# Daffan/legged_tracking

Measured on AMD Instinct MI355X. Metric: env-steps/sec (whole node) at 4096 Go1/GPU, 1/2/4/8 MI355X; %HBM roofline, higher is better.
Workload: dtype f32

## Files before the change

legged_tracking_amd/csrc/go1_contact.h:

```cpp
#pragma once
#ifndef GO1_DEVICE_H
#error "include go1_device.h: its parts are not self-contained"
#endif
#pragma clang fp contract(on)

#define PSZX 20
#define PSZY 16
static_assert(PSZY == 16 && PSZX % 2 == 0, "the LDS-DMA patch staging maps 2 rows of 16 cells to a wave");
struct Terr {
  const float* tile;
  int nx, ny;
  float hs;
  const float2* patch;
  int pi0, pj0;
};

__device__ __forceinline__ float tile_at(const Terr& T, int layer, int i, int j) {
  i = min(max(i, 0), T.nx - 1);
  j = min(max(j, 0), T.ny - 1);
  return T.tile[((size_t)layer * T.nx + i) * T.ny + j];
}

struct CP {
  float k, d, kf, mu;
// ... 311 lines not shown
      ymin = fminf(ymin, pp[1]); ymax = fmaxf(ymax, pp[1]);
    }
    float sn, cn;
    __sincosf(q[j], &sn, &cn);
#pragma unroll
    for (int a = 0; a < 3; ++a) rE(j == 0 ? 0 : 1, cn, sn, Rp + 3 * a, Rp + 3 * a);
  }
  float fw[3];
  mat3_vec(Rp, GO1_MODEL_F32 + 13 * 10 + 4 * 9, fw);
  const float fx = pp[0] + fw[0], fy = pp[1] + fw[1];
  xmin = quad_min(fminf(xmin, fx)); xmax = quad_max(fmaxf(xmax, fx));
  ymin = quad_min(fminf(ymin, fy)); ymax = quad_max(fmaxf(ymax, fy));
  *cx = 0.5f * (xmin + xmax);
  *cy = 0.5f * (ymin + ymax);
}

#define FACE_Q 1.0e-5f
#define FACE_W 10
__device__ __forceinline__ int face_key_max(int v) {
  v = max(v, __builtin_amdgcn_update_dpp(0, v, 0xB1, 0xF, 0xF, true));
  v = max(v, __builtin_amdgcn_update_dpp(0, v, 0x4E, 0xF, 0xF, true));
  auto a = __builtin_amdgcn_permlane16_swap((uint32_t)v, (uint32_t)v, false, false);
  v = max((int)a[0], (int)a[1]);
  auto b = __builtin_amdgcn_permlane32_swap((uint32_t)v, (uint32_t)v, false, false);
  return max((int)b[0], (int)b[1]);
}
#define FACE_SIGNED 0.1f
__device__ __forceinline__ void face_scan(const Terr& T, const float* R, const float* pos, const float* th, int sub16,
                                          int* sel) {
  const float ihs = frcp(T.hs);
  const int ci = (int)floorf(fminf(fmaxf(pos[0] * ihs, -16000.0f), 16000.0f));
  const int cj = (int)floorf(fminf(fmaxf(pos[1] * ihs, -16000.0f), 16000.0f));
  int key[2] = {-1, -1};
#pragma unroll
  for (int u = 0; u < (FACE_W * FACE_W + 15) / 16; ++u) {
    const int v = sub16 + 16 * u;
    const int i = ci + v % FACE_W - 4, j = cj + v / FACE_W - 4;
    const int li = i - T.pi0, lj = j - T.pj0;
    const bool inp = (v < FACE_W * FACE_W) & (li >= 0) & (li < PSZX) & (lj >= 0) & (lj < PSZY);
    const float2 hv = T.patch[min(max(li, 0), PSZX - 1) * PSZY + min(max(lj, 0), PSZY - 1)];
    const float dx = (float)i * T.hs - pos[0], dy = (float)j * T.hs - pos[1];
    const f2 dz = f2{hv.x, hv.y} - pos[2];
    const f2 cx = (R[0] * dx + R[3] * dy) + R[6] * dz, cy = (R[1] * dx + R[4] * dy) + R[7] * dz,
             cz = (R[2] * dx + R[5] * dy) + R[8] * dz;
    const f2 pen = f2{cz.x + th[2], th[2] - cz.y};
#pragma unroll
    for (int hh = 0; hh < 2; ++hh) {
      const bool in = inp & (fabsf(cx[hh]) <= th[0]) & (fabsf(cy[hh]) <= th[1]) & (pen[hh] > -FACE_SIGNED);
      const int q = (int)floorf(fminf(pen[hh] + FACE_SIGNED, 10.0f) * (1.0f / FACE_Q));
      const int k = in ? (q << 7) | (127 - v) : -1;
      key[hh] = max(key[hh], k);
    }
  }
#pragma unroll
  for (int hh = 0; hh < 2; ++hh) {
    const int k = face_key_max(key[hh]);
    const int v = 127 - (k & 127);
    const int i = ci + v % FACE_W - 4, j = cj + v / FACE_W - 4;
    sel[hh] = k < 0 ? -1 : ((i + 16384) << 16) | (j + 16384);
  }
}
__device__ __forceinline__ void face_force(const Terr& T, const CP& C, const float* R, const float* pos, const float* vb,
                                           const float* th, const int* sel, f2* w, float* Fw) {
  f2 cx, cy, cz;
  bool ok[2];
#pragma unroll
  for (int hh = 0; hh < 2; ++hh) {
    const int i = (sel[hh] >> 16) - 16384, j = (sel[hh] & 0xffff) - 16384;
    const int li = i - T.pi0, lj = j - T.pj0;
    ok[hh] = sel[hh] >= 0 & li >= 0 & li < PSZX & lj >= 0 & lj < PSZY;
    const float2 hv = T.patch[min(max(li, 0), PSZX - 1) * PSZY + min(max(lj, 0), PSZY - 1)];
    const float dx = (float)i * T.hs - pos[0], dy = (float)j * T.hs - pos[1], dz = (hh == 0 ? hv.x : hv.y) - pos[2];
    cx[hh] = (R[0] * dx + R[3] * dy) + R[6] * dz;
// ... 30 lines not shown
```

legged_tracking_amd/csrc/go1_phys.h:

```cpp
#pragma once
#ifndef GO1_DEVICE_H
#error "include go1_device.h: its parts are not self-contained"
#endif
#pragma clang fp contract(on)

#define LDS_DDP (GO1_MODEL_FLOATS)
#define LDS_DPL (LDS_DDP + 12)
#define LDS_TL (LDS_DPL + 24)
#define LDS_HL (LDS_TL + 12)
#define LDS_GX (LDS_HL + 24)
#define LDS_GY (LDS_GX + GO1_GRID_X)
#define LDS_FLOATS (LDS_GY + GO1_GRID_Y)
static_assert(offsetof(go1_config, height_grid_y) - offsetof(go1_config, default_dof_pos) ==
                  (LDS_GY - LDS_DDP) * sizeof(float),
              "per-joint config arrays must be contiguous in go1_config");

struct Phys {
  float pos[3], quat[4];
  f2 wv[3];
  float q[3], qd[3];
};

__device__ __forceinline__ void phys_substep(CCfg* __restrict__ cfg, const float* lds, Phys& S, const float* tau,
                                             float h, const float* g, float friction, float restitution,
                                             float payload, const Terr& T, int leg, int role, bool cf_out,
                                             float* cf_raw, float* self_sc, bool face_scan_now) {
#pragma clang fp contract(on)
  (void)lds;
  const float* model = GO1_MODEL_F32;
  const float msx = (leg & 2) ? -1.0f : 1.0f, msy = (leg & 1) ? -1.0f : 1.0f, msxy = msx * msy;
  float LC[39];
#pragma unroll
  for (int i = 0; i < 39; ++i) {
    const int p = GO1_LEG_SIGN[i];
    LC[i] = p == 0 ? GO1_LEG_FL[i] : GO1_LEG_FL[i] * (p == 1 ? msx : (p == 2 ? msy : msxy));
  }
  MARK(phys_begin);
  const CP C = {cfg->contact_stiffness, cfg->contact_damping, cfg->friction_damping, friction,
                0.5f * (restitution + cfg->terrain_restitution), cfg->bounce_threshold};
  float R[9];
  quat_to_R(S.quat, R);
  f2 vbp[3];
#pragma unroll
  for (int i = 0; i < 3; ++i) vbp[i] = R[i] * S.wv[0] + R[3 + i] * S.wv[1] + R[6 + i] * S.wv[2];
  const float vb[6] = {vbp[0].x, vbp[1].x, vbp[2].x, vbp[0].y, vbp[1].y, vbp[2].y};
  const float* th = model + 13 * 10 + 4 * 9 + 3 + 1;
#ifndef GO1_ABL_NO_FACES
  if (T.patch && face_scan_now) {
    int sel[2];
    face_scan(T, R, S.pos, th, 4 * role + leg, sel);
    if (role == 0 && leg == 0) {
      int* fsel = reinterpret_cast<int*>(self_sc + FACE_SEL_OFF);
      fsel[0] = sel[0];
      fsel[1] = sel[1];
    }
    asm volatile("s_waitcnt lgkmcnt(0)" ::: "memory");
  }
#endif
  const float* origin = LC + 30;
  const float* foot = model + 13 * 10 + 4 * 9;
  const float foot_r = foot[3];
  const float thigh_r = model[13 * 10 + 4 * 9 + 3 + 1 + 3];
  const float calf_r = model[13 * 10 + 4 * 9 + 3 + 1 + 3 + 1];
  const float hip_r = model[13 * 10 + 4 * 9 + 3 + 1 + 3 + 2];
  const float hip_y0 = model[13 * 10 + 4 * 9 + 3 + 1 + 3 + 3], hip_y1 = model[13 * 10 + 4 * 9 + 3 + 1 + 3 + 4];
  float cs[3][2];
  const bool even = (role & 1) == 0;
  f2 Rs[9], ps[3], vs[6];
#pragma unroll
  for (int i = 0; i < 9; ++i) Rs[i] = f2{0.0f, R[i]};
#pragma unroll
  for (int i = 0; i < 3; ++i) { ps[i] = f2{0.0f, S.pos[i]}; vs[i] = f2{0.0f, vb[i]}; vs[3 + i] = f2{0.0f, vb[3 + i]}; }
  float pth[3], pkn[3], pft[3];
  f2 cjp[3][3], pAp[3][3];
  {
    f2 R01[3], pp01 = f2{S.pos[0], S.pos[1]};
    float R2[3], pp2 = S.pos[2];
    f2 vp[3];
#pragma unroll
    for (int k = 0; k < 3; ++k) { R01[k] = f2{R[k], R[3 + k]}; R2[k] = R[6 + k]; }
#pragma unroll
    for (int i = 0; i < 3; ++i) vp[i] = vbp[i];
#pragma unroll
    for (int j = 0; j < 3; ++j) {
      const int ax = j == 0 ? 0 : 1;
      const float* r = origin + j * 3;
      float sn, cn;
      hw_sincosf(S.q[j], &sn, &cn);
      cs[j][0] = cn; cs[j][1] = sn;
      f2 vj[3];
// ... 44 lines not shown
#pragma unroll
      for (int i = 0; i < 3; ++i) vp[i] = vj[i];
    }
  }
  MARK(leg_kin_done);
  float fx[6], fy[6], fbase[6];
  f2 Fpt[3];
  float Fo[3] = {0.0f, 0.0f, 0.0f};
  float Fbs[3] = {0.0f, 0.0f, 0.0f};
  SIP cin[2];
#ifndef GO1_ABL_NO_CONTACT
  {
    f2 lpA[3], lpB[3], rr;
    {
      const float* kn = origin + 6;
      const int cA = leg * 2, cB = leg * 2 + 1;
      const float crn[2][3] = {{(cA & 1) ? th[0] : -th[0], (cA & 2) ? th[1] : -th[1], (cA & 4) ? th[2] : -th[2]},
                               {(cB & 1) ? th[0] : -th[0], (cB & 2) ? th[1] : -th[1], (cB & 4) ? th[2] : -th[2]}};
#pragma unroll
      for (int i = 0; i < 3; ++i) {
        const float hyA = i == 1 ? msy * hip_y0 : 0.0f, hyB = i == 1 ? msy * hip_y1 : 0.0f;
        const float xa = sel4(role, 0.0f, hyA, 0.0f, foot[i]);
        const float xb = sel4(role, 0.5f * kn[i], hyB, 0.5f * foot[i], foot[i]);
        const float ya = sel4(role, kn[i], crn[0][i], foot[i], crn[1][i]);
        const float yb = sel4(role, 0.5f * kn[i], crn[0][i], 0.5f * foot[i], crn[1][i]);
        lpA[i] = f2{xa, ya};
        lpB[i] = f2{xb, yb};
      }
      rr = f2{sel4(role, thigh_r, hip_r, calf_r, foot_r), sel4(role, thigh_r, 0.0f, calf_r, 0.0f)};
    }
    float wb[6] = {0.0f, 0.0f, 0.0f, 0.0f, 0.0f, 0.0f}, Mo[3] = {0.0f, 0.0f, 0.0f};
    MARK(self_begin);
#ifndef GO1_ABL_NO_SELF
    const bool self_on = cfg->self_stiffness > 0.0f;
    int mask;
    {
      const f2 hy = msy * f2{hip_y0, hip_y1};
      const f2 hcy = origin[1] + cs[0][0] * hy, hcz = origin[2] + cs[0][1] * hy;
      const float hc0[3] = {origin[0], hcy.x, hcz.x}, hc1[3] = {origin[0], hcy.y, hcz.y};
      mask = self_broad(leg, pth, pkn, pft, fmaxf(foot_r, fmaxf(thigh_r, calf_r)), hc0, hc1, hip_r, R, S.pos, th,
                        S.q);
      mask = self_on ? mask : 0;
    }
#else
    const bool self_on = false;
    const int mask = 0;
#endif
    MARK(self_broad_done);
#ifdef GO1_ABL_NO_NARROW
    if (__any(mask != 0) && mask == 12345) {
#else
    if (__any(mask != 0)) {
#endif
      float P0[3], P1[3];
      f2 e[3];
      {
        const float* kn = origin + 6;
#pragma unroll
        for (int i = 0; i < 3; ++i) {
          const float hy0 = i == 1 ? msy * hip_y0 : 0.0f, hy1 = i == 1 ? msy * hip_y1 : 0.0f;
          e[i] = f2{sel4(role, 0.0f, hy0, 0.0f, foot[i]), sel4(role, kn[i], hy1, foot[i], foot[i])};
        }
#pragma unroll
        for (int i = 0; i < 3; ++i) {
          const f2 p = ps[i].x + Rs[3 * i].x * e[0] + Rs[3 * i + 1].x * e[1] + Rs[3 * i + 2].x * e[2];
          P0[i] = p.x; P1[i] = p.y;
        }
// ... 2 lines not shown
        const float w[3] = {vs[0].x, vs[1].x, vs[2].x};
        const f2 wl[3] = {w[1] * e[2] - w[2] * e[1], w[2] * e[0] - w[0] * e[2], w[0] * e[1] - w[1] * e[0]};
        const f2 vlin[3] = {vs[3].x + wl[0], vs[4].x + wl[1], vs[5].x + wl[2]};
#pragma unroll
        for (int i = 0; i < 3; ++i) {
          const f2 v = Rs[3 * i].x * vlin[0] + Rs[3 * i + 1].x * vlin[1] + Rs[3 * i + 2].x * vlin[2];
          V0[i] = v.x; V1[i] = v.y;
        }
      };
      const float half = sel4(role, 0.5f * fabsf(origin[8]), 0.5f * (hip_y1 - hip_y0), 0.5f * fabsf(foot[2]), 0.0f);
      self_put(self_sc, leg, role, P0, P1, rr.x, half + rr.x);
      static_assert(TPB == 64, "self-collision LDS exchange assumes one wave per block");
      asm volatile("s_waitcnt lgkmcnt(0)" ::: "memory");
      MARK(self_put_done);
      const float pb[3] = {ps[0].x, ps[1].x, ps[2].x};
      float own_lo[3], own_hi[3];
#pragma unroll
      for (int i = 0; i < 3; ++i) { own_lo[i] = fminf(P0[i], P1[i]) - rr.x; own_hi[i] = fmaxf(P0[i], P1[i]) + rr.x; }
      self_narrow(cfg, self_sc, leg, role, mask, R, S.pos, vb, th, pb, own_lo, own_hi, Fo, Mo, wb, vel);
      asm volatile("s_waitcnt lgkmcnt(0)" ::: "memory");
      MARK(self_narrow_done);
    }
    f2 lp[3], pw[3], vw[3];
    HQ qa, qb;
    int cell[2];
    {
      f2 wA[3], wB[3];
#pragma unroll
      for (int i = 0; i < 3; ++i) {
        wA[i] = ps[i] + Rs[3 * i] * lpA[0] + Rs[3 * i + 1] * lpA[1] + Rs[3 * i + 2] * lpA[2];
        wB[i] = ps[i] + Rs[3 * i] * lpB[0] + Rs[3 * i + 1] * lpB[1] + Rs[3 * i + 2] * lpB[2];
      }
      MARK(seg_begin);
      float2* held = reinterpret_cast<float2*>(self_sc + SEG_T_OFF) + (4 * role + leg);
      f2 ts;
      if (face_scan_now) {
#ifdef GO1_ABL_NO_WALK
        ts = f2{0.0f, 0.0f} * (wA[0] + wB[0]);
        cell[0] = SEG_CELL((int)floorf(wA[0].x / T.hs), (int)floorf(wA[1].x / T.hs), false);
        cell[1] = SEG_CELL((int)floorf(wA[0].y / T.hs), (int)floorf(wA[1].y / T.hs), false);
#else
        ts = seg_deepest2(T, wA, wB, rr, cell);
#endif
        *held = make_float2(ts.x, ts.y);
      } else {
        const float2 hv = *held;
        ts = f2{hv.x, hv.y};
      }
      MARK(seg_done);
#pragma unroll
      for (int i = 0; i < 3; ++i) lp[i] = lpA[i] + ts * (lpB[i] - lpA[i]);
      const f2 wl[3] = {vs[1] * lp[2] - vs[2] * lp[1], vs[2] * lp[0] - vs[0] * lp[2], vs[0] * lp[1] - vs[1] * lp[0]};
      const f2 vlin[3] = {vs[3] + wl[0], vs[4] + wl[1], vs[5] + wl[2]};
#pragma unroll
      for (int i = 0; i < 3; ++i) {
        pw[i] = ps[i] + Rs[3 * i] * lp[0] + Rs[3 * i + 1] * lp[1] + Rs[3 * i + 2] * lp[2];
        vw[i] = Rs[3 * i] * vlin[0] + Rs[3 * i + 1] * vlin[1] + Rs[3 * i + 2] * vlin[2];
      }
    }
    if (face_scan_now) {
      hq_fetch_cell(T, pw[0].x, pw[1].x, cell[0], qa);
      hq_fetch_cell(T, pw[0].y, pw[1].y, cell[1], qb);
    } else {
      hq_fetch(T, pw[0].x, pw[1].x, qa);
      hq_fetch(T, pw[0].y, pw[1].y, qb);
    }
    float Fa[3], Fb2[3], Ma[6], Mb[6];
    {
      const float pa[3] = {pw[0].x, pw[1].x, pw[2].x}, va[3] = {vw[0].x, vw[1].x, vw[2].x};
      const float pb[3] = {pw[0].y, pw[1].y, pw[2].y}, vb2[3] = {vw[0].y, vw[1].y, vw[2].y};
      sphere_contact_im(T, qa, C, pa, va, rr.x, h, Fa, Ma);
      sphere_contact_im(T, qb, C, pb, vb2, rr.y, h, Fb2, Mb);
    }
    if (self_on) {
#pragma unroll
      for (int i = 0; i < 3; ++i) Fbs[i] = R[3 * i] * wb[3] + R[3 * i + 1] * wb[4] + R[3 * i + 2] * wb[5];
    }
    const f2 F[3] = {f2{Fa[0], Fb2[0]}, f2{Fa[1], Fb2[1]}, f2{Fa[2], Fb2[2]}};
    f2 Fd[3];
#pragma unroll
// ... 156 lines not shown
      for (int a = 0; a < 3; ++a)
#pragma unroll
        for (int b = 0; b < 3; ++b) Ia.b[a * 3 + b] = IA.b[a * 3 + b] - Up[j][a].x * V[b].y;
      f2 Iac[3], pa[3], pt[3];
      sip_mul_sparse(Ia, cjp[j], ax, Iac);
      const float ud = u[j] * invD;
#pragma unroll
      for (int i = 0; i < 3; ++i) pa[i] = pAp[j][i] + Iac[i] + Up[j][i] * ud;
      SIP It;
      xform_inertia2(ax, cs[j][0], cs[j][1], offset_mask(j), origin + j * 3, Ia, It);
      xfT2(ax, cs[j][0], cs[j][1], offset_mask(j), origin + j * 3, pa, pt);
      if (j > 0) {
        rigid_sip(LC + 10 * (j - 1), 1.0f, IA);
        sip_add(IA, It);
        sip_add(IA, j == 2 ? ci_th : ci_hp);
#pragma unroll
        for (int i = 0; i < 3; ++i) pAp[j - 1][i] += pt[i];
      } else {
        Ip = It;
        sip_add(Ip, ci_bs);
#pragma unroll
        for (int i = 0; i < 3; ++i) pp6[i] = pt[i];
      }
    }
  }
  MARK(backward_done);
  f2 wface[3] = {f2{0.0f, 0.0f}, f2{0.0f, 0.0f}, f2{0.0f, 0.0f}};
  float Fface[3] = {0.0f, 0.0f, 0.0f};
#ifdef GO1_ABL_NO_FACES
  if (false) {
#else
  if (T.patch) {
#endif
    const int* fsel = reinterpret_cast<const int*>(self_sc + FACE_SEL_OFF);
    const int sel[2] = {fsel[0], fsel[1]};
    face_force(T, C, R, S.pos, vb, th, sel, wface, Fface);
  }
  MARK(faces_done);
  const float* bb = model;
  const float mscale = (bb[0] + payload) * frcp(bb[0]);
  SIP I0;
  rigid_sip(bb, mscale, I0);
  f2 p0[3];
  float gb[3];
  rigid_bias2(bb, vbp, p0, mscale);
  mat3T_vec(R, g, gb);
#pragma unroll
  for (int k = 0; k < 6; ++k) Ip.ac[k] = f2{qsum(Ip.ac[k].x), qsum(Ip.ac[k].y)};
#pragma unroll
  for (int i = 0; i < 3; ++i) pp6[i] = f2{qsum(pp6[i].x - fbase[i]), qsum(pp6[i].y - fbase[3 + i])} - wface[i];
#pragma unroll
  for (int i = 0; i < 9; ++i) Ip.b[i] = qsum(Ip.b[i]);
  sip_add(I0, Ip);
  float rhs[6], a0[6];
#pragma unroll
  for (int i = 0; i < 3; ++i) {
    rhs[i] = -(p0[i].x + pp6[i].x);
    rhs[3 + i] = -(p0[i].y + pp6[i].y);
  }
#ifdef GO1_ABL_NO_BASESOLVE
#pragma unroll
  for (int i = 0; i < 6; ++i) a0[i] = rhs[i] * 0.05f;
  (void)I0;
#else
#ifdef GO1_ABL_NO_CHOL
  float tr = 0.0f;
#pragma unroll
  for (int k = 0; k < 6; ++k) tr += I0.ac[k].x + I0.ac[k].y;
#pragma unroll
// ... 96 lines not shown
```

legged_tracking_amd/csrc/go1_selfcol.h:

```cpp
#pragma once
#ifndef GO1_DEVICE_H
#error "include go1_device.h: its parts are not self-contained"
#endif
#pragma clang fp contract(on)

#define SELF_ENV_FLOATS (16 * 16 + 4 + 32)
#define FACE_SEL_OFF (16 * 16)
#define SEG_T_OFF (16 * 16 + 4)

__device__ __forceinline__ void self_put(float* sc, int leg, int role, const float* P0, const float* P1, float r,
                                         float rb) {
  float4* Q = reinterpret_cast<float4*>(sc) + 4 * (4 * leg + role);
  Q[0] = make_float4(P0[0], P0[1], P0[2], r);
  Q[1] = make_float4(P1[0], P1[1], P1[2], rb);
}
__device__ __forceinline__ void self_put_vel(float* sc, int leg, int role, const float* V0, const float* V1) {
  float4* Q = reinterpret_cast<float4*>(sc) + 4 * (4 * leg + role);
  Q[2] = make_float4(V0[0], V0[1], V0[2], 0.0f);
  Q[3] = make_float4(V1[0], V1[1], V1[2], 0.0f);
}

__device__ __forceinline__ void seg_closest(const float* P0, const float* d1, const float* Q0, const float* d2,
                                            float& s, float& t) {
  const float r[3] = {P0[0] - Q0[0], P0[1] - Q0[1], P0[2] - Q0[2]};
  const float a = d1[0] * d1[0] + d1[1] * d1[1] + d1[2] * d1[2], e = d2[0] * d2[0] + d2[1] * d2[1] + d2[2] * d2[2];
  const float b = d1[0] * d2[0] + d1[1] * d2[1] + d1[2] * d2[2];
  const float c = d1[0] * r[0] + d1[1] * r[1] + d1[2] * r[2], f = d2[0] * r[0] + d2[1] * r[1] + d2[2] * r[2];
  float n[3], m[3];
  cross3(d1, d2, n);
  cross3(d2, r, m);
  const float den = n[0] * n[0] + n[1] * n[1] + n[2] * n[2], num = n[0] * m[0] + n[1] * m[1] + n[2] * m[2];
  const bool pa = a > 1e-12f, pe = e > 1e-12f;
  const float ia = pa ? frcp(a) : 0.0f, ie = pe ? frcp(e) : 0.0f;
  const float s0 = den > 1e-10f * a * e ? __builtin_amdgcn_fmed3f(num * frcp(den), 0.0f, 1.0f) : 0.0f;
  const float tt = (b * s0 + f) * ie;
  const float s_lo = __builtin_amdgcn_fmed3f(-c * ia, 0.0f, 1.0f), s_hi = __builtin_amdgcn_fmed3f((b - c) * ia, 0.0f, 1.0f);
  const float ss = tt < 0.0f ? s_lo : (tt > 1.0f ? s_hi : s0);
  const float t_pt = __builtin_amdgcn_fmed3f(f * ie, 0.0f, 1.0f);
  s = !pa ? 0.0f : (!pe ? s_lo : ss);
  t = !pe ? 0.0f : (!pa ? t_pt : __builtin_amdgcn_fmed3f(tt, 0.0f, 1.0f));
}
// ... 274 lines not shown
```

legged_tracking_amd/csrc/go1_spec.h:

```cpp
#pragma once
#define GO1_SPEC_FIELDS(X) \
  X(terrain_kind, 1) \
  X(camera_zero, 1) \
  X(measure_front_half, 1) \
  X(add_noise, 1) \
  X(use_terminal_body_height, 1) \
  X(rand_interval, 300) \
  X(hf_nx, 80) \
  X(hf_ny, 40) \
  X(n_terms, 10) \
  X(term_mask, 23647u) \
  X(reward_mode, 0) \
  X(lin_vel_form, 0) \
  X(terminate_end_of_trajectory, 0) \
  X(use_terminal_body_rotation, 0) \
  X(rotate_camera, 0) \
  X(observe_heights, 1) \
  X(timestep_in_obs, 0) \
  X(num_obs, 261) \
  X(u_per_env, 308) \
  X(traj_kind, 0) \
  X(traj_length, 1) \
  X(traj_interp, 1) \
  X(indefinite_slots, 0u) \
  X(live_slots, 1023u) \
  X(sigma_rew_neg, 0x1.4000000000000p+2f) \
  X(small_vel_threshold, 0x1.99999a0000000p-4f) \
  X(large_dist_threshold, 0x0.0p+0f) \
  X(dt, 0x1.47ae140000000p-6f) \
  X(action_scale, 0x1.0000000000000p-2f) \
  X(hip_scale_reduction, 0x1.0000000000000p-1f) \
  X(clip_actions, 0x1.4000000000000p+3f) \
  X(clip_obs, 0x1.9000000000000p+6f) \
  X(horizontal_scale, 0x1.99999a0000000p-5f) \
// ... 33 lines not shown
#define GO1_SPEC_action_scale 0x1.0000000000000p-2f
#define GO1_SPEC_hip_scale_reduction 0x1.0000000000000p-1f
#define GO1_SPEC_clip_actions 0x1.4000000000000p+3f
#define GO1_SPEC_clip_obs 0x1.9000000000000p+6f
#define GO1_SPEC_horizontal_scale 0x1.99999a0000000p-5f
#define GO1_SPEC_max_episode_length 0x1.f400000000000p+8f
#define GO1_SPEC_terminal_body_height 0x0.0p+0f
#define GO1_SPEC_switch_dist 0x1.3333340000000p-2f
#define GO1_SPEC_base_height_target 0x1.1eb8520000000p-2f
#define GO1_SPEC_tracking_sigma_lin 0x1.99999a0000000p-5f
#define GO1_SPEC_tracking_sigma_ang 0x1.0000000000000p-1f
#define GO1_SPEC_target_lin_vel 0x1.0000000000000p-2f
#define GO1_SPEC_target_ang_vel 0x1.921fb60000000p+0f
#define GO1_SPEC_lin_reaching_criterion 0x1.3333340000000p-2f
#define GO1_SPEC_ang_reaching_criterion 0x1.41b2f80000000p-3f
#define GO1_SPEC_t_reach 0x0.0p+0f
#define GO1_SPEC_ceiling_height 0x1.99999a0000000p-1f
#define GO1_SPEC_obs_scale_dof_pos 0x1.0000000000000p+0f
#define GO1_SPEC_obs_scale_dof_vel 0x1.99999a0000000p-5f
#define GO1_SPEC_obs_scale_heights 0x1.99999a0000000p-4f
#define GO1_SPEC_noise_gravity 0x1.99999a0000000p-5f
#define GO1_SPEC_noise_dof_pos 0x1.47ae140000000p-7f
#define GO1_SPEC_noise_dof_vel 0x1.3333340000000p-4f
#define GO1_SPEC_camera_offset_x 0x1.eb851e0000000p-4f
#define GO1_SPEC_camera_offset_norm 0x1.eb851e0000000p-4f
#define GO1_SPEC_priv_friction_shift 0x1.0000000000000p-1f
#define GO1_SPEC_priv_friction_scale 0x1.0000000000000p+1f
#define GO1_SPEC_priv_rest_shift 0x1.0000000000000p-1f
#define GO1_SPEC_priv_rest_scale 0x1.0000000000000p+1f
#define GO1_SPEC_strength_range 0x1.99999a0000000p-3f
#define GO1_SPEC_strength_lo 0x1.cccccc0000000p-1f
#define GO1_SPEC_offset_range 0x1.47ae140000000p-5f
#define GO1_SPEC_offset_lo -0x1.47ae140000000p-6f
#define GO1_SPEC_terrain_kind 1
#define GO1_SPEC_camera_zero 1
#define GO1_SPEC_measure_front_half 1
#define GO1_SPEC_add_noise 1
#define GO1_SPEC_use_terminal_body_height 1
#define GO1_SPEC_rand_interval 300
#define GO1_SPEC_hf_nx 80
#define GO1_SPEC_hf_ny 40
#define GO1_SPEC_n_terms 10
#define GO1_SPEC_term_mask 23647u
#define GO1_SPEC_reward_mode 0
#define GO1_SPEC_lin_vel_form 0
#define GO1_SPEC_terminate_end_of_trajectory 0
#define GO1_SPEC_use_terminal_body_rotation 0
#define GO1_SPEC_rotate_camera 0
#define GO1_SPEC_observe_heights 1
#define GO1_SPEC_timestep_in_obs 0
#define GO1_SPEC_num_obs 261
#define GO1_SPEC_u_per_env 308
#define GO1_SPEC_traj_kind 0
#define GO1_SPEC_traj_length 1
#define GO1_SPEC_traj_interp 1
#define GO1_SPEC_indefinite_slots 0u
#define GO1_SPEC_live_slots 1023u
```

legged_tracking_amd/csrc/go1_step.hip:

```cpp
#include "go1_device.h"
#include "go1_step_shared.h"

#define HOLD_N 23

struct KArgs {
  go1_state st;
  go1_terrain ter;
  go1_step_args a;
  int32_t* flags;
  int cur, prv, nxt;
  const uint8_t* prev_time_out;
  uint8_t* prev_extras;
  float* bucket_r;
  double* bucket_sum;
};

__device__ void traj_waypoint(CCfg* __restrict__ c, const Rng& rng, const float* root, int w, float* o) {
  const int ub = GO1_U_NOISE + c->num_obs;
  if (c->traj_kind == 1) {
    const int ni = c->traj_interp, nt = c->traj_length / ni + 1, sg = w / ni, j = w % ni;
    const float rng_of[6] = {c->traj_x_range, c->traj_y_range, c->traj_z_range, c->traj_yaw_range,
                             c->traj_pitch_range, c->traj_roll_range};
    const int out_of[6] = {0, 1, 2, 5, 4, 3};
#pragma unroll
// ... 211 lines not shown
        const int tix_s = __builtin_amdgcn_readlane(tix, 4 * el2);
        const int pi_s = __builtin_amdgcn_readlane(T.pi0, 4 * el2);
        const int pj_s = __builtin_amdgcn_readlane(T.pj0, 4 * el2);
        const float* tl = K.ter.tiles + (size_t)tix_s * 2 * nx * ny;
        const int gj = min(max(pj_s + cj, 0), ny - 1);
#pragma unroll
        for (int k = 0; k < PSZX / 2; ++k) {
          const int gi = min(max(pi_s + 2 * k + ci_l, 0), nx - 1);
          __builtin_amdgcn_global_load_lds(tl + (layer_off + gi) * ny + gj, (float*)&s_patch[el2][0] + 64 * k, 4, 0, 0);
        }
      }
    }
  }
  MARK(pro_dma_issued);
  __shared__ float s_hold[HOLD_N][TPB];
  auto hold = [&](bool park) {
    int hl = lane;
    if (!park) asm volatile("" : "+v"(hl));
    float* hp = &s_hold[0][hl];
    auto f = [&](int k, float& v) { if (park) hp[k * TPB] = v; else v = hp[k * TPB]; };
    auto i = [&](int k, int& v) { float x = __int_as_float(v); f(k, x); v = __float_as_int(x); };
#pragma unroll
    for (int k = 0; k < 6; ++k) f(k, traj_in[k]);
#pragma unroll
    for (int k = 0; k < 3; ++k) { f(6 + k, ldv[k]); f(9 + k, la[k]); f(12 + k, eo_pre[k]); }
    f(15, cam_pitch); f(16, my_scale); f(17, my_sum); f(18, my_tot);
    i(19, ep_in); i(20, idx_in); i(21, coll_in); i(22, my_id);
  };
  hold(true);
  asm volatile("" : "+v"(rebind_flag));
  if (rebind && sub16 == 0 && rebind_flag) K.prev_extras[e] = rebind_val;

  float cf_raw[CF_RAW] = {0, 0, 0, 0, 0, 0, 0, 0, 0}, cf_leg[9], cf_base[3], cf_hip[3];
  step_substeps<INJ>(c, A, J, P, s_mlp, s_phys, T, s_self[el], cf_raw, KL, friction, restitution, payload, e, lane,
                     CI(action_scale), CI(hip_scale_reduction), leg, role);
  contact_totals<INJ>(cf_raw, A.inj_contact, e, leg, role, cf_leg, cf_base, cf_hip);
  hold(false);
  float root[13];
  if (INJ) {
#pragma unroll
    for (int i = 0; i < 13; ++i) root[i] = A.inj_root[(size_t)e * 13 + i];
  } else {
    phys_store_root(P, root);
    root[0] = P.pos[0] + org_x;
    root[1] = P.pos[1] + org_y;
  }
  const bool hplane = CI(terrain_kind) == 0;
  const float scan_x = root[0], scan_y = root[1];
  const float cam_p = CI(rotate_camera) ? 0.0f : cam_pitch;
  float camx = 0.0f, camy = 0.0f;
  if (!hplane) {
    const float cos_p = pm_cosf(cam_p);
    camx = CI(camera_offset_x) * cos_p;
    camy = 0.0f * cos_p;
  }
  auto sample = [&](int i, int j, float& h0, float& h1) {
    if (hplane) { h0 = 1.0f; h1 = 0.0f; return; }
    float px, py;
    if constexpr (STREAM) {
      px = c_gen->scan_x[i] + scan_x;
      py = c_gen->scan_y[j] + scan_y;
    } else {
      px = s_phys[LDS_GX + i] + scan_x;
      py = s_phys[LDS_GY + j] + scan_y;
    }
    if (CI(camera_zero)) { px = px + camx; py = py + camy; }
    px = px - org_x;
    py = py - org_y;
    const float fx = fminf(fmaxf(px / CI(horizontal_scale), -1.0f), (float)CI(hf_nx));
    const float fy = fminf(fmaxf(py / CI(horizontal_scale), -1.0f), (float)CI(hf_ny));
// ... 536 lines not shown
  go1_terrain ter;
  bool bound = false, has_terrain = false;
  int32_t* d_flags = nullptr;
  float* d_bucket_r = nullptr;
  double* d_bucket_sum = nullptr;
  uint64_t count = 0;
  bool spec = false;
  bool streamed = false;
  const uint8_t* prev_time_out = nullptr;
  uint8_t* prev_extras = nullptr;
};

static thread_local std::string g_err;

#define P(f, cols, dt) GO1_PLANE(go1_state, f, cols, GO1_DTYPE_##dt)
static const PlaneRow STATE_PLANES[] = {
    P(root, 13, F32), P(dof_pos, 12, F32), P(dof_vel, 12, F32), P(last_actions, 12, F32), P(last_dof_vel, 12, F32),
    P(lag, 0, F32), P(pos_err_hist, 24, F32), P(vel_hist, 24, F32), P(motor_strength, 12, F32),
    P(motor_offset, 12, F32), P(friction, 1, F32), P(restitution, 1, F32), P(payload, 1, F32),
    P(episode_length, 1, I32), P(curr_pose_index, 1, I32), P(trajectory, 0, F32), P(base_rotation, 3, F32),
    P(collision_count, 1, I32), P(episode_sums, 0, F32), P(joint_pos_target, 12, F32), P(feet_air_time, 4, F32),
    P(last_contacts, 4, F32)};
#undef P
static_assert(sizeof(STATE_PLANES) / sizeof(STATE_PLANES[0]) == GO1_STATE_PLANES &&
                  sizeof(go1_state) == GO1_STATE_PLANES * sizeof(void*), "go1_state planes");

template <class T>
static bool spec_eq(T a, T b) { return memcmp(&a, &b, sizeof(T)) == 0; }
static bool spec_match(const go1_config& c) {
  bool m = true;
#define GO1_SPEC_CHECK(f, v) m = m && spec_eq(c.f, (decltype(c.f))(v));
  GO1_SPEC_FIELDS(GO1_SPEC_CHECK)
#undef GO1_SPEC_CHECK
  return m && c.decimation == 4;
}
static bool scan_compiled_in(const go1_config& c) { return c.scan_nx == GO1_GRID_X && c.scan_ny == GO1_GRID_Y; }

static int fail(int code, const std::string& msg) {
  g_err = msg;
  return code;
}
#define HIP_TRY(x) GO1_HIP_TRY(fail, x)
int go1_internal_fail(int code, const std::string& msg) { return fail(code, msg); }

extern "C" {
#ifdef GO1_STAMPS
int go1_debug_stamps(void* host, size_t bytes) {
  if (bytes > sizeof(g_go1_stamps)) bytes = sizeof(g_go1_stamps);
  return hipMemcpyFromSymbol(host, HIP_SYMBOL(g_go1_stamps), bytes, 0, hipMemcpyDeviceToHost) == hipSuccess ? 0 : 1;
}
int go1_debug_stamps_clear(void) {
  void* p = nullptr;
  if (hipGetSymbolAddress(&p, HIP_SYMBOL(g_go1_stamps)) != hipSuccess) return 1;
  if (hipMemset(p, 0, sizeof(g_go1_stamps)) != hipSuccess) return 1;
  return hipDeviceSynchronize() == hipSuccess ? 0 : 1;
}
#endif

int go1_abi_version(void) { return GO1_ABI_VERSION; }

void go1_abi_sizes(int64_t out[4]) {
  out[0] = sizeof(go1_config);
  out[1] = sizeof(go1_state);
  out[2] = sizeof(go1_terrain);
  out[3] = sizeof(go1_step_args);
}

// ... 236 lines not shown
```

legged_tracking_amd/csrc/go1_step_shared.h:

```cpp
#pragma once
#include "go1_device.h"

#pragma clang fp contract(off)

template <int KMAX>
struct Joints {
  float (&act)[3], (&q)[3], (&qd)[3], (&eh)[2][3], (&vh)[2][3], (&strength)[3], (&offset)[3];
  float (&dflt)[3], (&tlim)[3], (&lag_pre)[KMAX][3];
  float (&scaled)[3], (&torque)[3], (&tgt)[3];
};

__device__ __forceinline__ void phys_load_root(Phys& P, const float* root) {
#pragma unroll
  for (int i = 0; i < 3; ++i) {
    P.pos[i] = root[i];
    P.wv[i] = f2{root[10 + i], root[7 + i]};
  }
#pragma unroll
  for (int i = 0; i < 4; ++i) P.quat[i] = root[3 + i];
}
__device__ __forceinline__ void phys_store_root(const Phys& P, float* root) {
#pragma unroll
  for (int i = 0; i < 3; ++i) {
    root[i] = P.pos[i]; root[7 + i] = P.wv[i].y; root[10 + i] = P.wv[i].x;
  }
#pragma unroll
  for (int i = 0; i < 4; ++i) root[3 + i] = P.quat[i];
}

template <bool INJ, int KMAX, class Args>
__device__ __forceinline__ void step_substeps(CCfg* c, const Args& A, const Joints<KMAX>& J, Phys& P,
                                              const float* s_mlp, const float* s_phys, const Terr& T, float* s_self,
                                              float* cf_raw, int KL, float friction, float restitution,
                                              float payload, int e, int lane, float action_scale,
                                              float hip_scale_reduction, int leg, int role) {
  const int lq = lane >> 4, n = c->n_envs, dec = c->decimation;
#pragma unroll
  for (int j = 0; j < 3; ++j) {
    J.scaled[j] = J.act[j] * action_scale;
    if (j == 0) J.scaled[j] = J.scaled[j] * hip_scale_reduction;
  }
  for (int sub = 0; sub < dec; ++sub) {
    MARK(sub_begin);
    {
      const int m = 6 - sub;
      const int back = m <= 0 ? 0 : (m + dec - 1) / dec;
      float xin[3][6];
#pragma unroll
      for (int j = 0; j < 3; ++j) {
        float lg = J.scaled[j];
#pragma unroll
        for (int k = 0; k < KMAX; ++k) lg = back == KL - k ? J.lag_pre[k][j] : lg;
        J.tgt[j] = lg + J.dflt[j];
        const float err = J.q[j] - J.tgt[j] + J.offset[j];
        xin[j][0] = err; xin[j][1] = J.eh[0][j]; xin[j][2] = J.eh[1][j];
        xin[j][3] = J.qd[j]; xin[j][4] = J.vh[0][j]; xin[j][5] = J.vh[1][j];
      }
      MARK(mlp_begin);
      float tq[3] = {0.0f, 0.0f, 0.0f};
      float b0[3], b1v[3];
#pragma unroll
      for (int j = 0; j < 3; ++j) {
        const float* y = xin[j];
        b0[j] = sel4(lq, y[0], y[1], y[2], y[3]);
        b1v[j] = sel4(lq, y[4], y[5], 0.0f, 0.0f);
      }
#ifdef GO1_ABL_NO_MLP
#pragma unroll
      for (int j = 0; j < 3; ++j) tq[j] = 0.0f * (b0[j] + b1v[j]);
#else
      {
        MlpFrag Fs;
        mlp_unpark(Fs, s_mlp, lane);
        mlp_group3(Fs, b0, b1v, tq);
      }
#endif
#ifdef GO1_ABL_NO_MLP
#pragma unroll
      for (int j = 0; j < 3; ++j) tq[j] += -20.0f * xin[j][0] - 0.5f * xin[j][3];
#endif
      MARK(mlp_done);
#pragma unroll
      for (int j = 0; j < 3; ++j) {
        J.eh[1][j] = J.eh[0][j];
        J.eh[0][j] = xin[j][0];
        J.vh[1][j] = J.vh[0][j];
        J.vh[0][j] = J.qd[j];
        const float t = tq[j] * J.strength[j];
        const float lim = J.tlim[j];
        J.torque[j] = clampf(t, -lim, lim);
      }
    }
    if (INJ) {
      const float* id = A.inj_dof + ((size_t)sub * n + e) * NDOF * 2;
#pragma unroll
      for (int j = 0; j < 3; ++j) {
        J.q[j] = id[(leg * 3 + j) * 2];
        J.qd[j] = id[(leg * 3 + j) * 2 + 1];
      }
    } else {
      const float h = c->sim_dt / (float)c->n_internal;
#pragma unroll
      for (int j = 0; j < 3; ++j) { P.q[j] = J.q[j]; P.qd[j] = J.qd[j]; }
      MARK(phys_call);
#ifndef GO1_ABL_NO_PHYS
      for (int k = 0; k < c->n_internal; ++k) {
        const bool last = (sub == dec - 1) && (k == c->n_internal - 1);
        phys_substep(c, s_phys, P, J.torque, h, A.sim_gravity, friction, restitution, payload, T, leg, role, last,
                     cf_raw, s_self, sub == 0 && k == 0);
      }
#else
      P.qd[0] += 1e-4f * J.torque[0]; P.qd[1] += 1e-4f * J.torque[1]; P.qd[2] += 1e-4f * J.torque[2];
#endif
#pragma unroll
      for (int j = 0; j < 3; ++j) { J.q[j] = P.q[j]; J.qd[j] = P.qd[j]; }
      MARK(phys_returned);
    }
    if (A.dbg_torques && role == 0) {
#pragma unroll
      for (int j = 0; j < 3; ++j) A.dbg_torques[((size_t)sub * n + e) * NDOF + leg * 3 + j] = J.torque[j];
    }
  }
}

template <bool INJ>
__device__ __forceinline__ void contact_totals(const float* cf_raw, const float* inj_contact, int e,
                                               int leg, int role, float* cf_leg, float* cf_base, float* cf_hip) {
  cf_sum(cf_raw, role, cf_leg, cf_base, cf_hip);
  if (INJ) {
    const float* ic = inj_contact + (size_t)e * NB * 3;
#pragma unroll
    for (int i = 0; i < 3; ++i) {
      cf_base[i] = ic[i];
      cf_hip[i] = ic[(1 + leg * 4) * 3 + i];
    }
#pragma unroll
    for (int b = 0; b < 3; ++b)
#pragma unroll
      for (int i = 0; i < 3; ++i) cf_leg[b * 3 + i] = ic[(2 + leg * 4 + b) * 3 + i];
  }
}
__device__ __forceinline__ void contact_store(float* out, int e, int leg, const float* cf_leg,
// ... 97 lines not shown
```

legged_tracking_amd/csrc/go1_velocity.hip:

```cpp
#include "go1_device.h"
#include "go1_step_shared.h"
#include "../../include/go1_velocity.h"

#include <algorithm>
#include <cstdlib>
#include <vector>

typedef const __attribute__((address_space(4))) go1_vel_config VCfg;
#define VLAG 2
#define SQRT2_F 1.41421353816986083984f
#define CAT_PRONK 0
#define CAT_TROT 1
#define CAT_PACE 2
#define CAT_BOUND 3

struct RngD {
  const double* U;
  uint64_t seed, step;
  int e, gid;
  __device__ double operator()(int slot) const {
    if (U) return U[(size_t)e * GO1_VEL_D_PER_ENV + slot];
    uint32_t c[4] = {(uint32_t)gid, 0x40000000u | ((uint32_t)slot >> 1), (uint32_t)step, (uint32_t)(step >> 32)};
    philox4x32(c, (uint32_t)seed, (uint32_t)(seed >> 32));
    const uint32_t a = c[2 * (slot & 1)] >> 5, b = c[2 * (slot & 1) + 1] >> 6;
// ... 159 lines not shown
#pragma unroll
    for (int k = 0; k < VLAG; ++k) lag_pre[k][j] = lag_in[k * 12 + j];
    ldv[j] = st.last_dof_vel[d0 + j];
    la[j] = st.last_actions[d0 + j];
    lla[j] = st.last_last_actions[d0 + j];
    ljpt[j] = st.last_joint_pos_target[d0 + j];
    lljpt[j] = st.last_last_joint_pos_target[d0 + j];
  }
  const float friction = st.friction[e], payload = st.payload[e], restitution = st.restitution[e];
  __shared__ __attribute__((aligned(16))) float s_self[SEPB][SELF_ENV_FLOATS];
  const float eo_pre[3] = {K.env_origins[(size_t)e * 3], K.env_origins[(size_t)e * 3 + 1],
                           K.env_origins[(size_t)e * 3 + 2]};
  const int ep_in = st.episode_length[e];
  const float gait_in = st.gait_indices[e];
  const float lc_in = st.last_contacts[(size_t)e * 4 + leg];
  const int cat_in = st.command_categories[e], bin_in = st.command_bins[e];
  const int NC = NT + GO1_VEL_SUM_EXTRA, NE = NT + 1;
  float cs[2], es[2];
  float my_scale[2];
  int my_id[2];
#pragma unroll
  for (int h = 0; h < 2; ++h) {
    const int k = sub16 + 16 * h;
    cs[h] = k < NC ? st.command_sums[(size_t)e * NC + k] : 0.0f;
    es[h] = k < NE ? st.episode_sums[(size_t)e * NE + k] : 0.0f;
    my_scale[h] = k < NT ? A.reward_scales[k] : 0.0f;
    my_id[h] = k < NT ? v_gen->term_ids[k] : -1;
  }
  Phys P;
  if (!INJ) phys_load_root(P, st.root + (size_t)e * 13);
  const Terr T = {nullptr, 0, 0, 1.0f, nullptr, 0, 0};

  float cf_raw[CF_RAW] = {0, 0, 0, 0, 0, 0, 0, 0, 0}, cf_leg[9], cf_base[3], cf_hip[3];
  step_substeps<INJ>(c, A, J, P, s_mlp, nullptr, T, s_self[el], cf_raw, VLAG, friction, restitution, payload, e, lane,
                     c->action_scale, c->hip_scale_reduction, leg, role);
  float cmd[GO1_VEL_NUM_COMMANDS];
#pragma unroll
  for (int k = 0; k < GO1_VEL_NUM_COMMANDS; ++k) cmd[k] = st.commands[(size_t)e * GO1_VEL_NUM_COMMANDS + k];
  float root[13], fp[3], fv[3];
  contact_totals<INJ>(cf_raw, A.inj_contact, e, leg, role, cf_leg, cf_base, cf_hip);
  if (INJ) {
#pragma unroll
    for (int i = 0; i < 13; ++i) root[i] = A.inj_root[(size_t)e * 13 + i];
    const float* ft = A.inj_feet + ((size_t)e * 4 + leg) * 6;
#pragma unroll
    for (int i = 0; i < 3; ++i) { fp[i] = ft[i]; fv[i] = ft[3 + i]; }
  } else {
    phys_store_root(P, root);
    foot_state(root, q, qd, leg, fp, fv);
  }
  if (A.contact_forces && owner) contact_store(A.contact_forces, e, leg, cf_leg, cf_base, cf_hip);

  const int ep = ep_in + 1;
  float blv[3], bav[3], pg[3];
  {
    const float qb[4] = {root[3], root[4], root[5], root[6]};
    quat_rotate_inverse_f(qb, root + 7, blv);
    quat_rotate_inverse_f(qb, root + 10, bav);
    quat_rotate_inverse_f(qb, A.gravity_vec, pg);
  }
  const float gait = remainder_f(gait_in + v->dt * cmd[4], 1.0f);
  float fi_raw;
  {
    const float ph = cmd[5], off = cmd[6], bnd = cmd[7];
    const float f0 = ((gait + ph) + off) + bnd, f1 = gait + off, f2_ = gait + bnd, f3 = gait + ph;
    fi_raw = sel4(leg, f0, f1, f2_, f3);
  }
  const float foot_idx = remainder_f(fi_raw, 1.0f);
// ... 1233 lines not shown
```

Baseline: 63.68 million.

## Keep substep state in registers, pin uniform constants to SGPRs, specialize decimation

Batches the face-scan patch loads ahead of the compute loop so LDS latency overlaps. Moves the per-leg face selection and held segment depths out of LDS scratch and into per-thread registers, which drops the LDS stores, loads and the explicit waitcnt. Hoists the contact constants and the timestep, pins them to scalar registers, and moves the MLP fragment unpark out of the inner substep. Decimation and the internal substep count become compile-time constants in the spec kernel. Holding these values per thread raises VGPR pressure, and the loop is now marked unroll 1, which may change occupancy.

```diff
diff --git a/legged_tracking_amd/csrc/go1_contact.h b/legged_tracking_amd/csrc/go1_contact.h
--- a/legged_tracking_amd/csrc/go1_contact.h
+++ b/legged_tracking_amd/csrc/go1_contact.h
@@ -367,13 +367,25 @@
   const int ci = (int)floorf(fminf(fmaxf(pos[0] * ihs, -16000.0f), 16000.0f));
   const int cj = (int)floorf(fminf(fmaxf(pos[1] * ihs, -16000.0f), 16000.0f));
   int key[2] = {-1, -1};
-#pragma unroll
-  for (int u = 0; u < (FACE_W * FACE_W + 15) / 16; ++u) {
+  constexpr int NU = (FACE_W * FACE_W + 15) / 16;
+  static_assert(NU == 7, "the operand list below");
+  float2 hw[NU];
+#pragma unroll
+  for (int u = 0; u < NU; ++u) {
+    const int v = sub16 + 16 * u;
+    const int li = ci + v % FACE_W - 4 - T.pi0, lj = cj + v / FACE_W - 4 - T.pj0;
+    hw[u] = T.patch[min(max(li, 0), PSZX - 1) * PSZY + min(max(lj, 0), PSZY - 1)];
+  }
+  asm volatile("" : "+v"(hw[0].x), "+v"(hw[0].y), "+v"(hw[1].x), "+v"(hw[1].y), "+v"(hw[2].x), "+v"(hw[2].y),
+                    "+v"(hw[3].x), "+v"(hw[3].y), "+v"(hw[4].x), "+v"(hw[4].y), "+v"(hw[5].x), "+v"(hw[5].y),
+                    "+v"(hw[6].x), "+v"(hw[6].y));
+#pragma unroll
+  for (int u = 0; u < NU; ++u) {
     const int v = sub16 + 16 * u;
     const int i = ci + v % FACE_W - 4, j = cj + v / FACE_W - 4;
     const int li = i - T.pi0, lj = j - T.pj0;
     const bool inp = (v < FACE_W * FACE_W) & (li >= 0) & (li < PSZX) & (lj >= 0) & (lj < PSZY);
-    const float2 hv = T.patch[min(max(li, 0), PSZX - 1) * PSZY + min(max(lj, 0), PSZY - 1)];
+    const float2 hv = hw[u];
     const float dx = (float)i * T.hs - pos[0], dy = (float)j * T.hs - pos[1];
     const f2 dz = f2{hv.x, hv.y} - pos[2];
     const f2 cx = (R[0] * dx + R[3] * dy) + R[6] * dz, cy = (R[1] * dx + R[4] * dy) + R[7] * dz,
diff --git a/legged_tracking_amd/csrc/go1_phys.h b/legged_tracking_amd/csrc/go1_phys.h
--- a/legged_tracking_amd/csrc/go1_phys.h
+++ b/legged_tracking_amd/csrc/go1_phys.h
@@ -21,7 +21,30 @@
   float q[3], qd[3];
 };
 
-__device__ __forceinline__ void phys_substep(CCfg* __restrict__ cfg, const float* lds, Phys& S, const float* tau,
+template <class V>
+__device__ __forceinline__ void pin_s(V& v) {
+  static_assert(sizeof(V) == 4, "one SGPR");
+  int s = __builtin_amdgcn_readfirstlane(__builtin_bit_cast(int, v));
+  asm volatile("" : "+s"(s));
+  v = __builtin_bit_cast(V, s);
+}
+struct PhysK {
+  float kc, dc, df, rest_t, bounce;
+  float self_k;
+};
+__device__ __forceinline__ PhysK sub_consts(CCfg* __restrict__ cfg) {
+  PhysK K = {cfg->contact_stiffness, cfg->contact_damping, cfg->friction_damping, cfg->terrain_restitution,
+             cfg->bounce_threshold, cfg->self_stiffness};
+  pin_s(K.kc); pin_s(K.dc); pin_s(K.df); pin_s(K.rest_t); pin_s(K.bounce); pin_s(K.self_k);
+  return K;
+}
+struct Held {
+  f2 ts;
+  int face[2];
+};
+
+__device__ __forceinline__ void phys_substep(CCfg* __restrict__ cfg, const PhysK& K, Held& H, const float* lds,
+                                             Phys& S, const float* tau,
                                              float h, const float* g, float friction, float restitution,
                                              float payload, const Terr& T, int leg, int role, bool cf_out,
                                              float* cf_raw, float* self_sc, bool face_scan_now) {
@@ -36,8 +59,7 @@
     LC[i] = p == 0 ? GO1_LEG_FL[i] : GO1_LEG_FL[i] * (p == 1 ? msx : (p == 2 ? msy : msxy));
   }
   MARK(phys_begin);
-  const CP C = {cfg->contact_stiffness, cfg->contact_damping, cfg->friction_damping, friction,
-                0.5f * (restitution + cfg->terrain_restitution), cfg->bounce_threshold};
+  const CP C = {K.kc, K.dc, K.df, friction, 0.5f * (restitution + K.rest_t), K.bounce};
   float R[9];
   quat_to_R(S.quat, R);
   f2 vbp[3];
@@ -46,16 +68,7 @@
   const float vb[6] = {vbp[0].x, vbp[1].x, vbp[2].x, vbp[0].y, vbp[1].y, vbp[2].y};
   const float* th = model + 13 * 10 + 4 * 9 + 3 + 1;
 #ifndef GO1_ABL_NO_FACES
-  if (T.patch && face_scan_now) {
-    int sel[2];
-    face_scan(T, R, S.pos, th, 4 * role + leg, sel);
-    if (role == 0 && leg == 0) {
-      int* fsel = reinterpret_cast<int*>(self_sc + FACE_SEL_OFF);
-      fsel[0] = sel[0];
-      fsel[1] = sel[1];
-    }
-    asm volatile("s_waitcnt lgkmcnt(0)" ::: "memory");
-  }
+  if (T.patch && face_scan_now) face_scan(T, R, S.pos, th, 4 * role + leg, H.face);
 #endif
   const float* origin = LC + 30;
   const float* foot = model + 13 * 10 + 4 * 9;
@@ -166,7 +179,7 @@
     float wb[6] = {0.0f, 0.0f, 0.0f, 0.0f, 0.0f, 0.0f}, Mo[3] = {0.0f, 0.0f, 0.0f};
     MARK(self_begin);
 #ifndef GO1_ABL_NO_SELF
-    const bool self_on = cfg->self_stiffness > 0.0f;
+    const bool self_on = K.self_k > 0.0f;
     int mask;
     {
       const f2 hy = msy * f2{hip_y0, hip_y1};
@@ -235,7 +248,6 @@
         wB[i] = ps[i] + Rs[3 * i] * lpB[0] + Rs[3 * i + 1] * lpB[1] + Rs[3 * i + 2] * lpB[2];
       }
       MARK(seg_begin);
-      float2* held = reinterpret_cast<float2*>(self_sc + SEG_T_OFF) + (4 * role + leg);
       f2 ts;
       if (face_scan_now) {
 #ifdef GO1_ABL_NO_WALK
@@ -245,10 +257,9 @@
 #else
         ts = seg_deepest2(T, wA, wB, rr, cell);
 #endif
-        *held = make_float2(ts.x, ts.y);
+        H.ts = ts;
       } else {
-        const float2 hv = *held;
-        ts = f2{hv.x, hv.y};
+        ts = H.ts;
       }
       MARK(seg_done);
 #pragma unroll
@@ -471,9 +482,7 @@
 #else
   if (T.patch) {
 #endif
-    const int* fsel = reinterpret_cast<const int*>(self_sc + FACE_SEL_OFF);
-    const int sel[2] = {fsel[0], fsel[1]};
-    face_force(T, C, R, S.pos, vb, th, sel, wface, Fface);
+    face_force(T, C, R, S.pos, vb, th, H.face, wface, Fface);
   }
   MARK(faces_done);
   const float* bb = model;
diff --git a/legged_tracking_amd/csrc/go1_selfcol.h b/legged_tracking_amd/csrc/go1_selfcol.h
--- a/legged_tracking_amd/csrc/go1_selfcol.h
+++ b/legged_tracking_amd/csrc/go1_selfcol.h
@@ -5,8 +5,6 @@
 #pragma clang fp contract(on)
 
 #define SELF_ENV_FLOATS (16 * 16 + 4 + 32)
-#define FACE_SEL_OFF (16 * 16)
-#define SEG_T_OFF (16 * 16 + 4)
 
 __device__ __forceinline__ void self_put(float* sc, int leg, int role, const float* P0, const float* P1, float r,
                                          float rb) {
diff --git a/legged_tracking_amd/csrc/go1_spec.h b/legged_tracking_amd/csrc/go1_spec.h
--- a/legged_tracking_amd/csrc/go1_spec.h
+++ b/legged_tracking_amd/csrc/go1_spec.h
@@ -1,5 +1,7 @@
 #pragma once
 #define GO1_SPEC_FIELDS(X) \
+  X(decimation, 4) \
+  X(n_internal, 1) \
   X(terrain_kind, 1) \
   X(camera_zero, 1) \
   X(measure_front_half, 1) \
@@ -99,6 +101,8 @@
 #define GO1_SPEC_strength_lo 0x1.cccccc0000000p-1f
 #define GO1_SPEC_offset_range 0x1.47ae140000000p-5f
 #define GO1_SPEC_offset_lo -0x1.47ae140000000p-6f
+#define GO1_SPEC_decimation 4
+#define GO1_SPEC_n_internal 1
 #define GO1_SPEC_terrain_kind 1
 #define GO1_SPEC_camera_zero 1
 #define GO1_SPEC_measure_front_half 1
diff --git a/legged_tracking_amd/csrc/go1_step.hip b/legged_tracking_amd/csrc/go1_step.hip
--- a/legged_tracking_amd/csrc/go1_step.hip
+++ b/legged_tracking_amd/csrc/go1_step.hip
@@ -267,10 +267,10 @@
   if (rebind && sub16 == 0 && rebind_flag) K.prev_extras[e] = rebind_val;
 
   float cf_raw[CF_RAW] = {0, 0, 0, 0, 0, 0, 0, 0, 0}, cf_leg[9], cf_base[3], cf_hip[3];
-  step_substeps<INJ>(c, A, J, P, s_mlp, s_phys, T, s_self[el], cf_raw, KL, friction, restitution, payload, e, lane,
-                     CI(action_scale), CI(hip_scale_reduction), leg, role);
+  step_substeps<INJ, SPEC>(c, A, J, P, s_mlp, s_phys, T, s_self[el], cf_raw, KL, friction, restitution, payload, e,
+                           lane, CI(action_scale), CI(hip_scale_reduction), leg, role, CI(decimation), CI(n_internal));
+  hold(false);
   contact_totals<INJ>(cf_raw, A.inj_contact, e, leg, role, cf_leg, cf_base, cf_hip);
-  hold(false);
   float root[13];
   if (INJ) {
 #pragma unroll
@@ -873,7 +873,8 @@
 #define GO1_SPEC_CHECK(f, v) m = m && spec_eq(c.f, (decltype(c.f))(v));
   GO1_SPEC_FIELDS(GO1_SPEC_CHECK)
 #undef GO1_SPEC_CHECK
-  return m && c.decimation == 4;
+  static_assert(GO1_LAG_STEPS(GO1_SPEC_decimation) == 2, "go1_step_kernel<SPEC>: KMAX = KL = 2");
+  return m;
 }
 static bool scan_compiled_in(const go1_config& c) { return c.scan_nx == GO1_GRID_X && c.scan_ny == GO1_GRID_Y; }
 
diff --git a/legged_tracking_amd/csrc/go1_step_shared.h b/legged_tracking_amd/csrc/go1_step_shared.h
--- a/legged_tracking_amd/csrc/go1_step_shared.h
+++ b/legged_tracking_amd/csrc/go1_step_shared.h
@@ -28,21 +28,31 @@
   for (int i = 0; i < 4; ++i) root[3 + i] = P.quat[i];
 }
 
-template <bool INJ, int KMAX, class Args>
+template <bool INJ, bool FIXED, int KMAX, class Args>
 __device__ __forceinline__ void step_substeps(CCfg* c, const Args& A, const Joints<KMAX>& J, Phys& P,
                                               const float* s_mlp, const float* s_phys, const Terr& T, float* s_self,
                                               float* cf_raw, int KL, float friction, float restitution,
                                               float payload, int e, int lane, float action_scale,
-                                              float hip_scale_reduction, int leg, int role) {
-  const int lq = lane >> 4, n = c->n_envs, dec = c->decimation;
+                                              float hip_scale_reduction, int leg, int role, int dec, int n_int) {
+  const int lq = lane >> 4, n = c->n_envs;
+  if (!FIXED) { pin_s(dec); pin_s(n_int); }
+  float h = c->sim_dt / (float)n_int;
+  pin_s(h);
+  const PhysK PK = sub_consts(c);
+  Held H = {f2{0.0f, 0.0f}, {-1, -1}};
 #pragma unroll
   for (int j = 0; j < 3; ++j) {
     J.scaled[j] = J.act[j] * action_scale;
     if (j == 0) J.scaled[j] = J.scaled[j] * hip_scale_reduction;
   }
+#pragma unroll 1
   for (int sub = 0; sub < dec; ++sub) {
     MARK(sub_begin);
     {
+#ifndef GO1_ABL_NO_MLP
+      MlpFrag Fs;
+      mlp_unpark(Fs, s_mlp, lane);
+#endif
       const int m = 6 - sub;
       const int back = m <= 0 ? 0 : (m + dec - 1) / dec;
       float xin[3][6];
@@ -69,11 +79,7 @@
 #pragma unroll
       for (int j = 0; j < 3; ++j) tq[j] = 0.0f * (b0[j] + b1v[j]);
 #else
-      {
-        MlpFrag Fs;
-        mlp_unpark(Fs, s_mlp, lane);
-        mlp_group3(Fs, b0, b1v, tq);
-      }
+      mlp_group3(Fs, b0, b1v, tq);
 #endif
 #ifdef GO1_ABL_NO_MLP
 #pragma unroll
@@ -99,15 +105,15 @@
         J.qd[j] = id[(leg * 3 + j) * 2 + 1];
       }
     } else {
-      const float h = c->sim_dt / (float)c->n_internal;
 #pragma unroll
       for (int j = 0; j < 3; ++j) { P.q[j] = J.q[j]; P.qd[j] = J.qd[j]; }
       MARK(phys_call);
 #ifndef GO1_ABL_NO_PHYS
-      for (int k = 0; k < c->n_internal; ++k) {
-        const bool last = (sub == dec - 1) && (k == c->n_internal - 1);
-        phys_substep(c, s_phys, P, J.torque, h, A.sim_gravity, friction, restitution, payload, T, leg, role, last,
-                     cf_raw, s_self, sub == 0 && k == 0);
+#pragma unroll 1
+      for (int k = 0; k < n_int; ++k) {
+        const bool last = (sub == dec - 1) && (k == n_int - 1);
+        phys_substep(c, PK, H, s_phys, P, J.torque, h, A.sim_gravity, friction, restitution, payload, T, leg, role,
+                     last, cf_raw, s_self, sub == 0 && k == 0);
       }
 #else
       P.qd[0] += 1e-4f * J.torque[0]; P.qd[1] += 1e-4f * J.torque[1]; P.qd[2] += 1e-4f * J.torque[2];
diff --git a/legged_tracking_amd/csrc/go1_velocity.hip b/legged_tracking_amd/csrc/go1_velocity.hip
--- a/legged_tracking_amd/csrc/go1_velocity.hip
+++ b/legged_tracking_amd/csrc/go1_velocity.hip
@@ -215,8 +215,8 @@
   const Terr T = {nullptr, 0, 0, 1.0f, nullptr, 0, 0};
 
   float cf_raw[CF_RAW] = {0, 0, 0, 0, 0, 0, 0, 0, 0}, cf_leg[9], cf_base[3], cf_hip[3];
-  step_substeps<INJ>(c, A, J, P, s_mlp, nullptr, T, s_self[el], cf_raw, VLAG, friction, restitution, payload, e, lane,
-                     c->action_scale, c->hip_scale_reduction, leg, role);
+  step_substeps<INJ, false>(c, A, J, P, s_mlp, nullptr, T, s_self[el], cf_raw, VLAG, friction, restitution, payload, e,
+                            lane, c->action_scale, c->hip_scale_reduction, leg, role, c->decimation, c->n_internal);
   float cmd[GO1_VEL_NUM_COMMANDS];
 #pragma unroll
   for (int k = 0; k < GO1_VEL_NUM_COMMANDS; ++k) cmd[k] = st.commands[(size_t)e * GO1_VEL_NUM_COMMANDS + k];
```

After: 64.69 million, median of 6. 1.02x the previous value.
